# Dhia-naouali/dinov3-jax

Measured on NVIDIA H100. Metric: global_crops_per_sec, higher is better.
Workload: dtype bf16

## Files before the change

### dinov3-jax_b200/csrc/attention.cu

```cuda
#include "ptx.cuh"
#include <climits>
#include <cstdlib>
#include "d3_internal.h"

namespace d3 {

constexpr float LOG2E = 1.4426950408889634f;
constexpr int SMEM_ALIGN = 1024;

__device__ __forceinline__ uint8_t* smem_base_1024(uint8_t* raw) {
  return reinterpret_cast<uint8_t*>((reinterpret_cast<uintptr_t>(raw) + 1023) & ~uintptr_t(1023));
}

struct AttnShape {
  int G;
  int span;
  int n_crops;
  int N;
  int nkb;
  int D;
  int H;
  float scale;
  const float* sin_t;
  const float* cos_t;
  int prefix;
};

__device__ __forceinline__ uint32_t sw128_offset(int row, int col) {
  return (uint32_t)(row * 128 + ((((col >> 3) ^ (row & 7)) & 7) << 4) + (col & 7) * 2);
}

struct RowInfo { int g, klo, khi; bool ok; };
__device__ __forceinline__ RowInfo row_info(const AttnShape& sh, int c, int q) {
  RowInfo ri;
  ri.g = min(q / sh.N, sh.G - 1);
  ri.klo = ri.g * sh.N;
  ri.khi = ri.klo + sh.N;
  ri.ok = (q < sh.span) && (c * sh.G + ri.g < sh.n_crops);
  return ri;
}

template <int NI, int NO>
__device__ __forceinline__ void online_softmax(float (&s)[4 * NI], float (&o)[NO], float (&m)[2], float (&l)[2],
                                               const RowInfo (&ri)[2], int k0, int c2, float cs) {
  const int kb0 = k0 + c2;
  const bool full = k0 >= max(ri[0].klo, ri[1].klo) && k0 + 8 * NI <= min(ri[0].khi, ri[1].khi);
  float mx[2] = {-3.0e38f, -3.0e38f};
#pragma unroll
  for (int i = 0; i < NI; ++i)
#pragma unroll
    for (int j = 0; j < 4; ++j) {
      const int hh = j >> 1, kk = kb0 + 8 * i + (j & 1);
      if (full || (kk >= ri[hh].klo && kk < ri[hh].khi)) mx[hh] = fmaxf(mx[hh], s[4 * i + j]);
    }
  float corr[2], ms[2];
#pragma unroll
  for (int hh = 0; hh < 2; ++hh) {
    mx[hh] = fmaxf(mx[hh], __shfl_xor_sync(0xffffffffu, mx[hh], 1));
    mx[hh] = fmaxf(mx[hh], __shfl_xor_sync(0xffffffffu, mx[hh], 2));
    const float mn = fmaxf(m[hh], mx[hh]);
    corr[hh] = ex2_approx((m[hh] - mn) * cs);
    m[hh] = mn;
    ms[hh] = mn * cs;
    l[hh] *= corr[hh];
  }
#pragma unroll
  for (int i = 0; i < NI; ++i)
#pragma unroll
    for (int j = 0; j < 4; ++j) {
      const int hh = j >> 1, kk = kb0 + 8 * i + (j & 1);
      const float p = (full || (kk >= ri[hh].klo && kk < ri[hh].khi)) ? ex2_approx(fmaf(s[4 * i + j], cs, -ms[hh])) : 0.f;
      s[4 * i + j] = p;
      l[hh] += p;
      if (i < NO / 4) o[4 * i + j] *= corr[hh];
    }
}

template <int NO>
__device__ __forceinline__ void store_o_lse(const float (&o)[NO], float (&l)[2], const float (&m)[2], const RowInfo (&ri)[2],
                                            const AttnShape& sh, int c, int h, int row_base, int wq0, int r_in, int c2,
                                            __nv_bfloat16* O, float* LSE) {
#pragma unroll
  for (int hh = 0; hh < 2; ++hh) {
    l[hh] += __shfl_xor_sync(0xffffffffu, l[hh], 1);
    l[hh] += __shfl_xor_sync(0xffffffffu, l[hh], 2);
    const int q = wq0 + r_in + 8 * hh;
    if (!ri[hh].ok) continue;
    const float inv = 1.f / l[hh];
    __nv_bfloat16* dst = O + (size_t)(row_base + q) * sh.D + h * (2 * NO) + c2;
#pragma unroll
    for (int i = 0; i < NO / 4; ++i)
      *reinterpret_cast<uint32_t*>(dst + 8 * i) = pack_bf16(o[4 * i + 2 * hh] * inv, o[4 * i + 2 * hh + 1] * inv);
    if (LSE && c2 == 0)
      LSE[((size_t)(c * sh.G + ri[hh].g) * sh.H + h) * sh.N + (q - ri[hh].klo)] = m[hh] * sh.scale + logf(l[hh]);
  }
}

__host__ __device__ constexpr int fwd_smem(int nkb) { return SMEM_ALIGN + 16384 + 2 * nkb * 8192 + 8; }

__global__ void __launch_bounds__(256)
attn_fwd_kernel(const __grid_constant__ CUtensorMap tmQ, const __grid_constant__ CUtensorMap tmKV,
                __nv_bfloat16* __restrict__ O, float* __restrict__ LSE, const AttnShape sh) {
  extern __shared__ uint8_t smem_raw[];
  uint8_t* sQ = smem_base_1024(smem_raw);
  uint8_t* sK = sQ + 16384;
  uint8_t* sV = sK + sh.nkb * 8192;
  uint64_t* bar = reinterpret_cast<uint64_t*>(sV + sh.nkb * 8192);

// ... 264 lines not shown
  const uint64_t kd = gmma_desc_sw128(smem_u32(sK), 16, 1024);
  const uint64_t vd = gmma_desc_sw128(smem_u32(sV), 16, 1024);
  wgmma_fence();
#pragma unroll
  for (int k = 0; k < 4; ++k) {
    wgmma_m64n128k16_ss<0, 0>(s, qd + 2 * k, kd + 2 * k, k > 0 ? 1u : 0u);
    wgmma_m64n128k16_ss<0, 0>(dp, dod + 2 * k, vd + 2 * k, k > 0 ? 1u : 0u);
  }
  wgmma_commit();
  wgmma_wait<0>();
  fence_regs(s);
  fence_regs(dp);
#pragma unroll
  for (int hh = 0; hh < 2; ++hh) {
    const int q = q0 + r_in + 8 * hh;
    const RowInfo ri = row_info(sh, c, q);
    float lse2, dl;
    row_stats(sh, LSE, Delta, c, h, q, lse2, dl);
    const int lo = ri.ok ? ri.klo - kt * 128 : 0, hi = ri.ok ? ri.khi - kt * 128 : 0;
#pragma unroll
    for (int i = 0; i < 16; ++i)
#pragma unroll
      for (int j = 0; j < 2; ++j) {
        const int e = 4 * i + 2 * hh + j, col = 8 * i + c2 + j;
        const bool ok = col >= lo && col < hi;
        const float p = ok ? ex2_approx(fmaf(s[e], cs, -lse2)) : 0.f;
        dp[e] = ok ? (p * sh.scale) * (dp[e] - dl) : 0.f;
        s[e] = p;
      }
  }
}

__device__ __forceinline__ void stash_p_ds(const float (&s)[64], const float (&dp)[64], uint8_t* sP, uint8_t* sDS, int row,
                                           int c2) {
#pragma unroll
  for (int hh = 0; hh < 2; ++hh) {
#pragma unroll
    for (int i = 0; i < 16; ++i) {
      const uint32_t off = (i >> 3) * 16384 + sw128_offset(row + 8 * hh, (8 * i + c2) & 63);
      *reinterpret_cast<uint32_t*>(sP + off) = pack_bf16(s[4 * i + 2 * hh], s[4 * i + 2 * hh + 1]);
      *reinterpret_cast<uint32_t*>(sDS + off) = pack_bf16(dp[4 * i + 2 * hh], dp[4 * i + 2 * hh + 1]);
    }
  }
}

__device__ __forceinline__ void dkdv_mma(float (&dk)[32], float (&dv)[32], const uint8_t* sP, const uint8_t* sDS,
                                         const uint8_t* sDOt, const uint8_t* sQt, int wg) {
  const uint64_t pd = gmma_desc_sw128(smem_u32(sP + wg * 16384), 16384, 1024);
  const uint64_t sd = gmma_desc_sw128(smem_u32(sDS + wg * 16384), 16384, 1024);
  const uint64_t dod = gmma_desc_sw128(smem_u32(sDOt), 8192, 1024);
  const uint64_t qd = gmma_desc_sw128(smem_u32(sQt), 8192, 1024);
  fence_regs(dk);
  fence_regs(dv);
  wgmma_fence();
#pragma unroll
  for (int k = 0; k < 8; ++k) {
    wgmma_m64n64k16_ss<1, 1>(dv, pd + 128 * k, dod + 128 * k, 1u);
    wgmma_m64n64k16_ss<1, 1>(dk, sd + 128 * k, qd + 128 * k, 1u);
  }
  wgmma_commit();
  wgmma_wait<0>();
  fence_regs(dk);
  fence_regs(dv);
}

__device__ __forceinline__ void dq_mma(float (&dq)[32], const float (&dp)[64], const uint8_t* sK) {
  uint32_t a[8][4];
#pragma unroll
  for (int kk = 0; kk < 8; ++kk)
#pragma unroll
    for (int e = 0; e < 4; ++e) a[kk][e] = pack_bf16(dp[8 * kk + 2 * e], dp[8 * kk + 2 * e + 1]);
  const uint64_t kd = gmma_desc_sw128(smem_u32(sK), 8192, 1024);
  fence_regs(dq);
  wgmma_fence();
#pragma unroll
  for (int kk = 0; kk < 8; ++kk) wgmma_m64n64k16_rs<1>(dq, a[kk], kd + 128 * kk, 1u);
  wgmma_commit();
  wgmma_wait<0>();
  fence_regs(dq);
}


__host__ __device__ constexpr int bwd_fused_smem(int n_t) {
  return n_t * 32768 * 2 + 32768 + (n_t > 1 ? 2 * 32768 : 0) + n_t * 128 * 8 + 2 * n_t * 8;
}

__device__ __forceinline__ uint64_t desc_here(const void* p, uint32_t lbo, uint32_t sbo) {
  uint32_t a;
  asm volatile("mov.b32 %0, %1;" : "=r"(a) : "r"(smem_u32(p)));
  return gmma_desc_sw128(a, lbo, sbo);
}

template <int R>
__device__ __forceinline__ void fence_frag(uint32_t (&a)[R][4]) {
#pragma unroll
  for (int i = 0; i < R; ++i)
#pragma unroll
    for (int e = 0; e < 4; ++e) asm volatile("" : "+r"(a[i][e])::"memory");
}

__global__ void __launch_bounds__(256, 1)
attn_bwd_fused_kernel(const __grid_constant__ CUtensorMap tmQKV, const __grid_constant__ CUtensorMap tmDO,
                      const float* __restrict__ LSE, const float* __restrict__ Delta, __nv_bfloat16* __restrict__ dQKV,
                      const AttnShape sh) {
  extern __shared__ __align__(1024) uint8_t smem_al[];
  const int nT = (sh.span + 127) / 128;
  uint8_t* sKV = smem_al;
  uint8_t* sQDO = sKV + nT * 32768;
  uint8_t* sDS = sQDO + nT * 32768;
  uint8_t* sDS0 = sDS + 32768;
  float* sDQ = reinterpret_cast<float*>(sDS0 + 32768);
  float* sLSE = reinterpret_cast<float*>(sDS + (nT > 1 ? 3 * 32768 : 32768));
  float* sDel = sLSE + nT * 128;
  uint64_t* bar_kv = reinterpret_cast<uint64_t*>(sDel + nT * 128);
  uint64_t* bar_q = bar_kv + nT;

  const int wg = threadIdx.x >> 7, t = threadIdx.x & 127;
  const int r_in = 16 * (t >> 5) + ((t & 31) >> 2), c2 = 2 * (t & 3);
  const int h = blockIdx.x, c = blockIdx.y;
  const int row_base = c * sh.span;
  if (threadIdx.x == 0) {
    tma_prefetch_desc(&tmQKV);
    tma_prefetch_desc(&tmDO);
    for (int i = 0; i < 2 * nT; ++i) mbar_init(bar_kv + i, 1);
    fence_mbar_init();
  }
  __syncthreads();
  if (threadIdx.x < 32 && elect_one()) {
    for (int i = 0; i < nT; ++i) {
      mbar_expect_tx(bar_kv + i, 32768);
      tma_load_2d(&tmQKV, bar_kv + i, sKV + i * 32768, sh.D + h * 64, row_base + i * 128);
      tma_load_2d(&tmQKV, bar_kv + i, sKV + i * 32768 + 16384, 2 * sh.D + h * 64, row_base + i * 128);
      mbar_expect_tx(bar_q + i, 32768);
      tma_load_2d(&tmQKV, bar_q + i, sQDO + i * 32768, h * 64, row_base + i * 128);
      tma_load_2d(&tmDO, bar_q + i, sQDO + i * 32768 + 16384, h * 64, row_base + i * 128);
    }
  }
  for (int q = threadIdx.x; q < nT * 128; q += 256) {
    const RowInfo ri = row_info(sh, c, q);
    const size_t stat = ((size_t)(c * sh.G + ri.g) * sh.H + h) * sh.N + (q - ri.klo);
    sLSE[q] = ri.ok ? LSE[stat] * LOG2E : 0.f;
    sDel[q] = ri.ok ? Delta[stat] : 0.f;
  }
  __syncthreads();

  const float cs = sh.scale * LOG2E;
  int pair = 0;
#pragma unroll 1
  for (int kt = 0; kt < nT; ++kt) {
    mbar_wait(bar_kv + kt, 0);
    const uint8_t* sK = sKV + kt * 32768;
    const uint8_t* sV = sK + 16384;
    int lo[2], hi[2];
#pragma unroll
    for (int hh = 0; hh < 2; ++hh) {
      const RowInfo ri = row_info(sh, c, kt * 128 + wg * 64 + r_in + 8 * hh);
      lo[hh] = ri.ok ? ri.klo : 0;
      hi[hh] = ri.ok ? ri.khi : 0;
    }
    float dk[32], dv[32];
#pragma unroll 1
    for (int qt = 0; qt < nT; ++qt, ++pair) {
      mbar_wait(bar_q + qt, 0);
      const uint8_t* sQt = sQDO + qt * 32768;
      const uint8_t* sDOt = sQt + 16384;
      const bool defer = nT == 2 && kt == 0 && qt == 0;
      uint8_t* stash = defer ? sDS0 : sDS;
      uint32_t pa[2][4][4], da[2][4][4];
#pragma unroll
      for (int hf = 0; hf < 2; ++hf) {
        float s[32], dp[32];
        {
          const uint64_t kd = desc_here(sK + wg * 8192, 16, 1024);
          const uint64_t vd = desc_here(sV + wg * 8192, 16, 1024);
          const uint64_t qd = desc_here(sQt + hf * 8192, 16, 1024);
          const uint64_t dod = desc_here(sDOt + hf * 8192, 16, 1024);
          wgmma_fence();
#pragma unroll
          for (int k = 0; k < 4; ++k) {
            wgmma_m64n64k16_ss<0, 0>(s, kd + 2 * k, qd + 2 * k, k > 0 ? 1u : 0u);
            wgmma_m64n64k16_ss<0, 0>(dp, vd + 2 * k, dod + 2 * k, k > 0 ? 1u : 0u);
          }
          wgmma_commit();
          wgmma_wait<0>();
          fence_regs(s);
          fence_regs(dp);
          if (hf == 1) { fence_frag(pa[0]); fence_frag(da[0]); }
        }
        const float* lse2 = sLSE + qt * 128 + hf * 64;
        const float* del = sDel + qt * 128 + hf * 64;
#pragma unroll
        for (int i = 0; i < 8; ++i) {
          const int col = 8 * i + c2;
          const float2 l2 = *reinterpret_cast<const float2*>(lse2 + col);
          const float2 dl = *reinterpret_cast<const float2*>(del + col);
          const int q = qt * 128 + hf * 64 + col;
          float pv[4], dv4[4];
#pragma unroll
          for (int j = 0; j < 4; ++j) {
            const int hh = j >> 1, qq = q + (j & 1);
            const bool ok = qq >= lo[hh] && qq < hi[hh];
            const float p = ok ? ex2_approx(fmaf(s[4 * i + j], cs, -((j & 1) ? l2.y : l2.x))) : 0.f;
            dv4[j] = ok ? (p * sh.scale) * (dp[4 * i + j] - ((j & 1) ? dl.y : dl.x)) : 0.f;
            pv[j] = p;
          }
          pa[hf][i >> 1][2 * (i & 1)] = pack_bf16(pv[0], pv[1]);
          pa[hf][i >> 1][2 * (i & 1) + 1] = pack_bf16(pv[2], pv[3]);
          da[hf][i >> 1][2 * (i & 1)] = pack_bf16(dv4[0], dv4[1]);
          da[hf][i >> 1][2 * (i & 1) + 1] = pack_bf16(dv4[2], dv4[3]);
        }
        if (hf == 0 && pair > 1) named_bar_sync(1, 256);
#pragma unroll
        for (int hh = 0; hh < 2; ++hh)
#pragma unroll
          for (int i = 0; i < 8; ++i) {
            const uint32_t off = hf * 16384 + sw128_offset(wg * 64 + r_in + 8 * hh, 8 * i + c2);
            *reinterpret_cast<uint32_t*>(stash + off) = da[hf][i >> 1][2 * (i & 1) + hh];
          }
        {
          const uint64_t dod = desc_here(sDOt, 8192, 1024);
          const uint64_t qd = desc_here(sQt, 8192, 1024);
          const uint32_t acc_on = (qt > 0 || hf > 0) ? 1u : 0u;
          if (acc_on) { fence_regs(dk); fence_regs(dv); }
          wgmma_fence();
#pragma unroll
          for (int kk = 0; kk < 4; ++kk) {
            const int ks = 4 * hf + kk;
            wgmma_m64n64k16_rs<1>(dv, pa[hf][kk], dod + 128 * ks, (acc_on || kk > 0) ? 1u : 0u);
            wgmma_m64n64k16_rs<1>(dk, da[hf][kk], qd + 128 * ks, (acc_on || kk > 0) ? 1u : 0u);
          }
          wgmma_commit();
        }
      }
      fence_proxy_async_smem();
      if (defer) {
        wgmma_wait<0>();
        fence_regs(dk);
        fence_regs(dv);
        fence_frag(pa[1]);
        fence_frag(da[1]);
        continue;
      }
      named_bar_sync(2, 256);
      const bool from_partial = nT == 2 && kt == 1 && qt == 1;
      float dq[32];
      float4* part = reinterpret_cast<float4*>(sDQ) + wg * 8 * 128 + t;
      if (from_partial) {
#pragma unroll
        for (int j = 0; j < 8; ++j) {
          const float4 v = part[j * 128];
          dq[4 * j] = v.x; dq[4 * j + 1] = v.y; dq[4 * j + 2] = v.z; dq[4 * j + 3] = v.w;
        }
      }
      {
        const uint64_t sd = desc_here(sDS + wg * 16384, 16384, 1024);
        const uint64_t kbd = desc_here(sK, 8192, 1024);
        fence_regs(dq);
        wgmma_fence();
#pragma unroll
        for (int kk = 0; kk < 8; ++kk)
          wgmma_m64n64k16_ss<1, 1>(dq, sd + 128 * kk, kbd + 128 * kk, (from_partial || kk > 0) ? 1u : 0u);
        if (nT == 2 && kt == 1 && qt == 0) {
          const uint64_t sd0 = desc_here(sDS0 + wg * 16384, 16384, 1024);
          const uint64_t k0d = desc_here(sKV, 8192, 1024);
#pragma unroll
          for (int kk = 0; kk < 8; ++kk) wgmma_m64n64k16_ss<1, 1>(dq, sd0 + 128 * kk, k0d + 128 * kk, 1u);
        }
        wgmma_commit();
        wgmma_wait<0>();
        fence_regs(dq);
        fence_regs(dk);
        fence_regs(dv);
        fence_frag(pa[1]);
        fence_frag(da[1]);
      }
      if (nT == 2 && kt == 0) {
#pragma unroll
        for (int j = 0; j < 8; ++j) part[j * 128] = make_float4(dq[4 * j], dq[4 * j + 1], dq[4 * j + 2], dq[4 * j + 3]);
      } else {
        store_grad_rows(dq, sh, c, row_base, qt * 128 + wg * 64, r_in, c2, h, 0, true, dQKV);
      }
    }
    store_grad_rows(dk, sh, c, row_base, kt * 128 + wg * 64, r_in, c2, h, 1, true, dQKV);
    store_grad_rows(dv, sh, c, row_base, kt * 128 + wg * 64, r_in, c2, h, 2, false, dQKV);
  }
}

using DkdvRing = TileRing<DKDV_STAGES, 32768>;
constexpr int DKDV_SMEM = SMEM_ALIGN + 2 * 16384 + 2 * 32768 + DkdvRing::SMEM + 8;
using DqRing = TileRing<DQ_STAGES, 32768>;
constexpr int DQ_SMEM = SMEM_ALIGN + 2 * 16384 + DqRing::SMEM + 8;

__global__ void __launch_bounds__(RING_THREADS, 1)
attn_bwd_dkdv_kernel(const __grid_constant__ CUtensorMap tmQKV, const __grid_constant__ CUtensorMap tmDO,
                     const float* __restrict__ LSE, const float* __restrict__ Delta, __nv_bfloat16* __restrict__ dQKV,
                     const AttnShape sh) {
  extern __shared__ uint8_t smem_raw[];
  uint8_t* sK = smem_base_1024(smem_raw);
  uint8_t* sV = sK + 16384;
  uint8_t* sP = sV + 16384;
  uint8_t* sDS = sP + 32768;
  const DkdvRing ring(sDS + 32768);
  uint64_t* bar_kv = ring.end();

  const int wg = threadIdx.x >> 7, t = threadIdx.x & 127;
  const int r_in = 16 * (t >> 5) + ((t & 31) >> 2), c2 = 2 * (t & 3);
  const int kt = blockIdx.x, h = blockIdx.y, c = blockIdx.z;
  const int row_base = c * sh.N, nq = (sh.N + 127) >> 7;
  if (threadIdx.x == 0) {
    tma_prefetch_desc(&tmQKV);
    tma_prefetch_desc(&tmDO);
    ring.init(8);
    mbar_init(bar_kv, 1);
    fence_mbar_init();
  }
  __syncthreads();
  if (ring_producer(wg, [&] {
        mbar_expect_tx(bar_kv, 32768);
        tma_load_2d(&tmQKV, bar_kv, sK, sh.D + h * 64, row_base + kt * 128);
        tma_load_2d(&tmQKV, bar_kv, sV, 2 * sh.D + h * 64, row_base + kt * 128);
        ring.fill(nq, [&](uint64_t* bar, uint8_t* dst, int qt) {
          tma_load_2d(&tmQKV, bar, dst, h * 64, row_base + qt * 128);
          tma_load_2d(&tmDO, bar, dst + 16384, h * 64, row_base + qt * 128);
        });
      }))
    return;
  mbar_wait(bar_kv, 0);
  float dk[32], dv[32];
#pragma unroll
  for (int i = 0; i < 32; ++i) { dk[i] = 0.f; dv[i] = 0.f; }
#pragma unroll 1
  for (int qt = 0; qt < nq; ++qt) {
    const uint8_t* sQt = ring.wait(qt);
    const uint8_t* sDOt = sQt + 16384;
    float s[64], dp[64];
    p_ds_tile(sh, LSE, Delta, c, h, qt * 128 + wg * 64, kt, sQt + wg * 8192, sDOt + wg * 8192, sK, sV, r_in, c2, s, dp);
    stash_p_ds(s, dp, sP, sDS, wg * 64 + r_in, c2);
    fence_proxy_async_smem();
    named_bar_sync(1, 256);
    dkdv_mma(dk, dv, sP, sDS, sDOt, sQt, wg);
    ring.release(qt);
    named_bar_sync(1, 256);
  }
  store_grad_rows(dk, sh, c, row_base, kt * 128 + wg * 64, r_in, c2, h, 1, true, dQKV);
  store_grad_rows(dv, sh, c, row_base, kt * 128 + wg * 64, r_in, c2, h, 2, false, dQKV);
}

__global__ void __launch_bounds__(RING_THREADS, 1)
attn_bwd_dq_kernel(const __grid_constant__ CUtensorMap tmQKV, const __grid_constant__ CUtensorMap tmDO,
                   const float* __restrict__ LSE, const float* __restrict__ Delta, __nv_bfloat16* __restrict__ dQKV,
                   const AttnShape sh) {
  extern __shared__ uint8_t smem_raw[];
  uint8_t* sQ = smem_base_1024(smem_raw);
  uint8_t* sDO = sQ + 16384;
  const DqRing ring(sDO + 16384);
  uint64_t* bar_q = ring.end();

  const int wg = threadIdx.x >> 7, t = threadIdx.x & 127;
  const int r_in = 16 * (t >> 5) + ((t & 31) >> 2), c2 = 2 * (t & 3);
  const int qt = blockIdx.x, h = blockIdx.y, c = blockIdx.z;
  const int q0 = qt * 128, row_base = c * sh.N, nk = (sh.N + 127) >> 7;
  const int n_wg = (q0 + 64 < sh.N) ? 2 : 1;
  if (threadIdx.x == 0) {
    tma_prefetch_desc(&tmQKV);
    tma_prefetch_desc(&tmDO);
    ring.init(4 * n_wg);
    mbar_init(bar_q, 1);
// ... 261 lines not shown
  int lo[2], hi[2];
#pragma unroll
  for (int hh = 0; hh < 2; ++hh) {
    const RowInfo ri = row_info(sh, c, wq0 + r_in + 8 * hh);
    row_stats(sh, LSE, Delta, c, h, wq0 + r_in + 8 * hh, lse2[hh], dl[hh]);
    lo[hh] = ri.ok ? ri.klo : 0;
    hi[hh] = ri.ok ? ri.khi : 0;
  }
  const float cs = sh.scale * LOG2E;
  float dq[64];
#pragma unroll
  for (int i = 0; i < 64; ++i) dq[i] = 0.f;
#pragma unroll 1
  for (int kt = 0; kt < nk; ++kt) {
    const uint8_t* sK = ring.wait(kt);
    const uint8_t* sV = sK + 32768;
#pragma unroll 1
    for (int hf = 0; hf < 2; ++hf) {
      float s[32], dp[32];
      wgmma_fence();
#pragma unroll
      for (int k = 0; k < 8; ++k) {
        wgmma_m64n64k16_ss<0, 0>(s, kdesc128(sQ + wg * 8192, k), kdesc128(sK + hf * 8192, k), k > 0 ? 1u : 0u);
        wgmma_m64n64k16_ss<0, 0>(dp, kdesc128(sDO + wg * 8192, k), kdesc128(sV + hf * 8192, k), k > 0 ? 1u : 0u);
      }
      wgmma_commit();
      wgmma_wait<0>();
      fence_regs(s);
      fence_regs(dp);
      uint32_t da[4][4];
#pragma unroll
      for (int i = 0; i < 8; ++i) {
        const int key = kt * 128 + hf * 64 + 8 * i + c2;
        float d4[4];
#pragma unroll
        for (int j = 0; j < 4; ++j) {
          const int hh = j >> 1, kk = key + (j & 1);
          const bool ok = kk >= lo[hh] && kk < hi[hh];
          const float p = ok ? ex2_approx(fmaf(s[4 * i + j], cs, -lse2[hh])) : 0.f;
          d4[j] = ok ? (p * sh.scale) * (dp[4 * i + j] - dl[hh]) : 0.f;
        }
        da[i >> 1][2 * (i & 1)] = pack_bf16(d4[0], d4[1]);
        da[i >> 1][2 * (i & 1) + 1] = pack_bf16(d4[2], d4[3]);
      }
      const uint64_t kd = desc_here(sK + hf * 8192, 16384, 1024);
      fence_regs(dq);
      wgmma_fence();
#pragma unroll
      for (int kk = 0; kk < 4; ++kk) wgmma_m64n128k16_rs<1>(dq, da[kk], kd + 128 * kk, 1u);
      wgmma_commit();
      wgmma_wait<0>();
      fence_regs(dq);
      fence_frag(da);
    }
    ring.release(kt);
  }
  store_grad_rows(dq, sh, c, row_base, wq0, r_in, c2, h, 0, true, dQKV);
}

static int make_map(CUtensorMap* map, const void* ptr, long rows, int cols, int ld, int box_rows) {
  cuuint64_t dims[2] = {(cuuint64_t)cols, (cuuint64_t)rows};
  cuuint64_t strides[1] = {(cuuint64_t)ld * 2};
  cuuint32_t box[2] = {64, (cuuint32_t)box_rows};
  cuuint32_t estr[2] = {1, 1};
  return encode_tensor_map_2d_bf16(map, ptr, dims, strides, box, estr);
}

constexpr int ATTN_MAX_TOKENS = 32768;
constexpr int ATTN_FWD_RESIDENT_SPAN = 448;
constexpr int ATTN_BWD_RESIDENT_SPAN = 256;

static int attn_shape(AttnShape* s, int n_crops, int N, int D, int H) {
  if (D != H * 64 && D != H * 128) return set_error(D3_ERR_ARG, "attention: head_dim must be 64 or 128");
  if (N <= 0 || n_crops <= 0) return set_error(D3_ERR_ARG, "attention: empty problem");
  if (N > ATTN_MAX_TOKENS) return set_error(D3_ERR_ARG, "attention: N > 32768 tokens per crop");
  if ((long)n_crops * N > INT_MAX) return set_error(D3_ERR_ARG, "attention: n_crops * N must be below 2^31 token rows");
  s->N = N; s->D = D; s->H = H; s->n_crops = n_crops;
  s->scale = (D == H * 64) ? 0.125f : 0.08838834764831845f;
  s->sin_t = nullptr; s->cos_t = nullptr; s->prefix = 0;
  s->G = (N <= 64) ? (128 / N) : 1;
  if (s->G > n_crops) s->G = n_crops;
  s->span = s->G * N;
  s->nkb = (s->span + 63) / 64;
  return D3_OK;
}

static int tile_grid(const AttnShape& s, dim3* grid) {
  const int groups = (s.n_crops + s.G - 1) / s.G;
  if (s.H > 65535 || groups > 65535) return set_error(D3_ERR_ARG, "attention: H and crop groups must be <= 65535");
  *grid = dim3((s.span + 127) / 128, s.H, groups);
  return D3_OK;
}

template <auto kernel, class... Args>
static int launch(dim3 grid, int threads, int smem, int smem_max, cudaStream_t st, const Args&... args) {
  static const cudaError_t cfg = cudaFuncSetAttribute(kernel, cudaFuncAttributeMaxDynamicSharedMemorySize, smem_max);
  (void)cfg;
  kernel<<<grid, threads, smem, st>>>(args...);
  D3_CHECK_LAUNCH();
  return D3_OK;
}

}

using namespace d3;

extern "C" {

int d3_attn_fwd(const void* qkv, void* o, float* lse, int n_crops, int N, int D, int H, void* stream) {
  AttnShape s;
  int rc = attn_shape(&s, n_crops, N, D, H);
  if (rc) return rc;
  dim3 grid;
  if ((rc = tile_grid(s, &grid))) return rc;
  const long T = (long)n_crops * N;
  cudaStream_t st = reinterpret_cast<cudaStream_t>(stream);
  __nv_bfloat16* out = (__nv_bfloat16*)o;
  CUtensorMap tqkv;
  if ((rc = make_map(&tqkv, qkv, T, 3 * D, 3 * D, 128))) return rc;
  if (D == H * 128)
    return launch<attn_fwd_hd128_kernel>(grid, RING_THREADS, HD128_FWD_SMEM, HD128_FWD_SMEM, st, tqkv, out, lse, s);
  if (s.span > ATTN_FWD_RESIDENT_SPAN)
    return launch<attn_fwd_stream_kernel>(grid, RING_THREADS, FWD_STREAM_SMEM, FWD_STREAM_SMEM, st, tqkv, out, lse, s);
  CUtensorMap tkv;
  if ((rc = make_map(&tkv, qkv, T, 3 * D, 3 * D, 64))) return rc;
  return launch<attn_fwd_kernel>(grid, 256, fwd_smem(s.nkb), fwd_smem((ATTN_FWD_RESIDENT_SPAN + 63) / 64), st, tqkv, tkv,
                                 out, lse, s);
}

int d3_attn_bwd(const void* qkv, const void* o, const void* d_o, const float* lse, float* delta_scratch, void* dqkv,
                int n_crops, int N, int D, int H, const float* rope_sin, const float* rope_cos, int rope_prefix,
                void* stream) {
  AttnShape s;
  int rc = attn_shape(&s, n_crops, N, D, H);
  if (rc) return rc;
  if ((rope_sin == nullptr) != (rope_cos == nullptr)) return set_error(D3_ERR_ARG, "d3_attn_bwd: sin/cos tables");
  if (!delta_scratch) return set_error(D3_ERR_ARG, "d3_attn_bwd: delta scratch buffer");
  const bool hd128 = D == H * 128;
  const bool streamed = s.span > ATTN_BWD_RESIDENT_SPAN;
  dim3 grid;
  if ((hd128 || streamed) && (rc = tile_grid(s, &grid))) return rc;
  s.sin_t = rope_sin; s.cos_t = rope_cos; s.prefix = rope_prefix;
  const long T = (long)n_crops * N;
  cudaStream_t st = reinterpret_cast<cudaStream_t>(stream);
  const long threads = T * (D / 8);
  if (hd128)
    attn_delta_kernel<128><<<(int)((threads + 255) / 256), 256, 0, st>>>((const __nv_bfloat16*)o, (const __nv_bfloat16*)d_o,
                                                                       delta_scratch, T, N, D, H);
  else
    attn_delta_kernel<64><<<(int)((threads + 255) / 256), 256, 0, st>>>((const __nv_bfloat16*)o, (const __nv_bfloat16*)d_o,
                                                                      delta_scratch, T, N, D, H);
  D3_CHECK_LAUNCH();
  CUtensorMap tqkv, tdo;
  if ((rc = make_map(&tqkv, qkv, T, 3 * D, 3 * D, 128))) return rc;
  if ((rc = make_map(&tdo, d_o, T, D, D, 128))) return rc;
  __nv_bfloat16* dq = (__nv_bfloat16*)dqkv;
  if (hd128) {
    if ((rc = launch<attn_bwd_dkdv_hd128_kernel>(grid, RING_THREADS, HD128_BWD_SMEM, HD128_BWD_SMEM, st, tqkv, tdo, lse,
                                                 delta_scratch, dq, s)))
      return rc;
    return launch<attn_bwd_dq_hd128_kernel>(grid, RING_THREADS, HD128_BWD_SMEM, HD128_BWD_SMEM, st, tqkv, tdo, lse,
                                            delta_scratch, dq, s);
  }
  if (streamed) {
    if ((rc = launch<attn_bwd_dkdv_kernel>(grid, RING_THREADS, DKDV_SMEM, DKDV_SMEM, st, tqkv, tdo, lse, delta_scratch, dq,
                                           s)))
      return rc;
    return launch<attn_bwd_dq_kernel>(grid, RING_THREADS, DQ_SMEM, DQ_SMEM, st, tqkv, tdo, lse, delta_scratch, dq, s);
  }
  return launch<attn_bwd_fused_kernel>(dim3(H, (n_crops + s.G - 1) / s.G), 256, bwd_fused_smem((s.span + 127) / 128),
                                       bwd_fused_smem(ATTN_BWD_RESIDENT_SPAN / 128), st, tqkv, tdo, lse, delta_scratch,
                                       dq, s);
}

}
```

Measured before the change: 550.0.

## Make fused attention backward persistent with double-buffered TMA prefetch of next item

The fused backward kernel becomes persistent: it launches at most one CTA per SM (by occupancy) and loops over (head, crop-group) items. Tile shared memory is fixed at two 64KB slots, so the next item's K/V/Q/dO tiles are TMA-loaded while the current one is computed. The next item's LSE/Delta stats are staged with cp.async. This is meant to hide per-CTA load latency and launch tail, at the cost of extra barriers, parity tracking and more complex slot reuse logic.

```diff
diff --git a/dinov3-jax_b200/csrc/attention.cu b/dinov3-jax_b200/csrc/attention.cu
--- a/dinov3-jax_b200/csrc/attention.cu
+++ b/dinov3-jax_b200/csrc/attention.cu
@@ -1,4 +1,5 @@
 #include "ptx.cuh"
+#include <algorithm>
 #include <climits>
 #include <cstdlib>
 #include "d3_internal.h"
@@ -24,6 +25,7 @@
   const float* sin_t;
   const float* cos_t;
   int prefix;
+  int items;
 };
 
 __device__ __forceinline__ uint32_t sw128_offset(int row, int col) {
@@ -454,7 +456,7 @@
 
 
 __host__ __device__ constexpr int bwd_fused_smem(int n_t) {
-  return n_t * 32768 * 2 + 32768 + (n_t > 1 ? 2 * 32768 : 0) + n_t * 128 * 8 + 2 * n_t * 8;
+  return 2 * 65536 + 32768 + (n_t > 1 ? 2 * 32768 : 0) + n_t * 128 * 8 + 2 * 8;
 }
 
 __device__ __forceinline__ uint64_t desc_here(const void* p, uint32_t lbo, uint32_t sbo) {
@@ -469,6 +471,38 @@
   for (int i = 0; i < R; ++i)
 #pragma unroll
     for (int e = 0; e < 4; ++e) asm volatile("" : "+r"(a[i][e])::"memory");
+}
+
+__device__ __forceinline__ void bwd_load_tile(const CUtensorMap* tmQKV, const CUtensorMap* tmDO, const AttnShape& sh,
+                                              int item, int tile, uint8_t* dst, uint64_t* bar) {
+  const int h = item % sh.H, row = (item / sh.H) * sh.span + tile * 128;
+  mbar_expect_tx(bar, 65536);
+  tma_load_2d(tmQKV, bar, dst, sh.D + h * 64, row);
+  tma_load_2d(tmQKV, bar, dst + 16384, 2 * sh.D + h * 64, row);
+  tma_load_2d(tmQKV, bar, dst + 32768, h * 64, row);
+  tma_load_2d(tmDO, bar, dst + 49152, h * 64, row);
+}
+
+__device__ __forceinline__ void bwd_stage_stats(const AttnShape& sh, const float* __restrict__ LSE,
+                                                const float* __restrict__ Delta, int item, int nT, float* sLSE,
+                                                float* sDel) {
+  const int h = item % sh.H, c = item / sh.H;
+  for (int q = threadIdx.x; q < nT * 128; q += 256) {
+    const RowInfo ri = row_info(sh, c, q);
+    const size_t stat = ((size_t)(c * sh.G + ri.g) * sh.H + h) * sh.N + (q - ri.klo);
+    if (ri.ok) {
+      cp_async_4(sLSE + q, LSE + stat);
+      cp_async_4(sDel + q, Delta + stat);
+    } else {
+      sLSE[q] = 0.f;
+      sDel[q] = 0.f;
+    }
+  }
+}
+
+__device__ __forceinline__ void bwd_stats_land(int nT, float* sLSE) {
+  cp_async_wait_all();
+  for (int q = threadIdx.x; q < nT * 128; q += 256) sLSE[q] *= LOG2E;
 }
 
 __global__ void __launch_bounds__(256, 1)
@@ -477,184 +511,195 @@
                       const AttnShape sh) {
   extern __shared__ __align__(1024) uint8_t smem_al[];
   const int nT = (sh.span + 127) / 128;
-  uint8_t* sKV = smem_al;
-  uint8_t* sQDO = sKV + nT * 32768;
-  uint8_t* sDS = sQDO + nT * 32768;
+  uint8_t* sT = smem_al;
+  uint8_t* sDS = sT + 2 * 65536;
   uint8_t* sDS0 = sDS + 32768;
   float* sDQ = reinterpret_cast<float*>(sDS0 + 32768);
   float* sLSE = reinterpret_cast<float*>(sDS + (nT > 1 ? 3 * 32768 : 32768));
   float* sDel = sLSE + nT * 128;
-  uint64_t* bar_kv = reinterpret_cast<uint64_t*>(sDel + nT * 128);
-  uint64_t* bar_q = bar_kv + nT;
+  uint64_t* bar = reinterpret_cast<uint64_t*>(sDel + nT * 128);
 
   const int wg = threadIdx.x >> 7, t = threadIdx.x & 127;
   const int r_in = 16 * (t >> 5) + ((t & 31) >> 2), c2 = 2 * (t & 3);
-  const int h = blockIdx.x, c = blockIdx.y;
-  const int row_base = c * sh.span;
   if (threadIdx.x == 0) {
     tma_prefetch_desc(&tmQKV);
     tma_prefetch_desc(&tmDO);
-    for (int i = 0; i < 2 * nT; ++i) mbar_init(bar_kv + i, 1);
+    mbar_init(bar, 1);
+    mbar_init(bar + 1, 1);
     fence_mbar_init();
   }
   __syncthreads();
-  if (threadIdx.x < 32 && elect_one()) {
-    for (int i = 0; i < nT; ++i) {
-      mbar_expect_tx(bar_kv + i, 32768);
-      tma_load_2d(&tmQKV, bar_kv + i, sKV + i * 32768, sh.D + h * 64, row_base + i * 128);
-      tma_load_2d(&tmQKV, bar_kv + i, sKV + i * 32768 + 16384, 2 * sh.D + h * 64, row_base + i * 128);
-      mbar_expect_tx(bar_q + i, 32768);
-      tma_load_2d(&tmQKV, bar_q + i, sQDO + i * 32768, h * 64, row_base + i * 128);
-      tma_load_2d(&tmDO, bar_q + i, sQDO + i * 32768 + 16384, h * 64, row_base + i * 128);
-    }
-  }
-  for (int q = threadIdx.x; q < nT * 128; q += 256) {
-    const RowInfo ri = row_info(sh, c, q);
-    const size_t stat = ((size_t)(c * sh.G + ri.g) * sh.H + h) * sh.N + (q - ri.klo);
-    sLSE[q] = ri.ok ? LSE[stat] * LOG2E : 0.f;
-    sDel[q] = ri.ok ? Delta[stat] : 0.f;
-  }
-  __syncthreads();
+  if (threadIdx.x == 0) {
+    bwd_load_tile(&tmQKV, &tmDO, sh, blockIdx.x, 0, sT, bar);
+    if (nT == 2) bwd_load_tile(&tmQKV, &tmDO, sh, blockIdx.x, 1, sT + 65536, bar + 1);
+    else if (blockIdx.x + gridDim.x < sh.items)
+      bwd_load_tile(&tmQKV, &tmDO, sh, blockIdx.x + gridDim.x, 0, sT + 65536, bar + 1);
+  }
+  bwd_stage_stats(sh, LSE, Delta, blockIdx.x, nT, sLSE, sDel);
 
   const float cs = sh.scale * LOG2E;
-  int pair = 0;
 #pragma unroll 1
-  for (int kt = 0; kt < nT; ++kt) {
-    mbar_wait(bar_kv + kt, 0);
-    const uint8_t* sK = sKV + kt * 32768;
-    const uint8_t* sV = sK + 16384;
-    int lo[2], hi[2];
-#pragma unroll
-    for (int hh = 0; hh < 2; ++hh) {
-      const RowInfo ri = row_info(sh, c, kt * 128 + wg * 64 + r_in + 8 * hh);
-      lo[hh] = ri.ok ? ri.klo : 0;
-      hi[hh] = ri.ok ? ri.khi : 0;
-    }
-    float dk[32], dv[32];
+  for (int it = 0; blockIdx.x + it * gridDim.x < sh.items; ++it) {
+    const int item = blockIdx.x + it * gridDim.x, next = item + gridDim.x;
+    const int h = item % sh.H, c = item / sh.H;
+    const int row_base = c * sh.span;
+    const uint32_t par = (nT == 1 ? it >> 1 : it) & 1;
+    bwd_stats_land(nT, sLSE);
+    __syncthreads();
+    int pair = 0;
 #pragma unroll 1
-    for (int qt = 0; qt < nT; ++qt, ++pair) {
-      mbar_wait(bar_q + qt, 0);
-      const uint8_t* sQt = sQDO + qt * 32768;
-      const uint8_t* sDOt = sQt + 16384;
-      const bool defer = nT == 2 && kt == 0 && qt == 0;
-      uint8_t* stash = defer ? sDS0 : sDS;
-      uint32_t pa[2][4][4], da[2][4][4];
-#pragma unroll
-      for (int hf = 0; hf < 2; ++hf) {
-        float s[32], dp[32];
+    for (int kt = 0; kt < nT; ++kt) {
+      const int kslot = nT == 1 ? (it & 1) : kt;
+      mbar_wait(bar + kslot, par);
+      const uint8_t* sK = sT + kslot * 65536;
+      const uint8_t* sV = sK + 16384;
+      int lo[2], hi[2];
+#pragma unroll
+      for (int hh = 0; hh < 2; ++hh) {
+        const RowInfo ri = row_info(sh, c, kt * 128 + wg * 64 + r_in + 8 * hh);
+        lo[hh] = ri.ok ? ri.klo : 0;
+        hi[hh] = ri.ok ? ri.khi : 0;
+      }
+      float dk[32], dv[32];
+#pragma unroll 1
+      for (int qt = 0; qt < nT; ++qt, ++pair) {
+        const int qslot = nT == 1 ? (it & 1) : qt;
+        mbar_wait(bar + qslot, par);
+        const uint8_t* sQt = sT + qslot * 65536 + 32768;
+        const uint8_t* sDOt = sQt + 16384;
+        const bool defer = nT == 2 && kt == 0 && qt == 0;
+        uint8_t* stash = defer ? sDS0 : sDS;
+        uint32_t pa[2][4][4], da[2][4][4];
+#pragma unroll
+        for (int hf = 0; hf < 2; ++hf) {
+          float s[32], dp[32];
+          {
+            const uint64_t kd = desc_here(sK + wg * 8192, 16, 1024);
+            const uint64_t vd = desc_here(sV + wg * 8192, 16, 1024);
+            const uint64_t qd = desc_here(sQt + hf * 8192, 16, 1024);
+            const uint64_t dod = desc_here(sDOt + hf * 8192, 16, 1024);
+            wgmma_fence();
+#pragma unroll
+            for (int k = 0; k < 4; ++k) {
+              wgmma_m64n64k16_ss<0, 0>(s, kd + 2 * k, qd + 2 * k, k > 0 ? 1u : 0u);
+              wgmma_m64n64k16_ss<0, 0>(dp, vd + 2 * k, dod + 2 * k, k > 0 ? 1u : 0u);
+            }
+            wgmma_commit();
+            wgmma_wait<0>();
+            fence_regs(s);
+            fence_regs(dp);
+            if (hf == 1) { fence_frag(pa[0]); fence_frag(da[0]); }
+          }
+          const float* lse2 = sLSE + qt * 128 + hf * 64;
+          const float* del = sDel + qt * 128 + hf * 64;
+#pragma unroll
+          for (int i = 0; i < 8; ++i) {
+            const int col = 8 * i + c2;
+            const float2 l2 = *reinterpret_cast<const float2*>(lse2 + col);
+            const float2 dl = *reinterpret_cast<const float2*>(del + col);
+            const int q = qt * 128 + hf * 64 + col;
+            float pv[4], dv4[4];
+#pragma unroll
+            for (int j = 0; j < 4; ++j) {
+              const int hh = j >> 1, qq = q + (j & 1);
+              const bool ok = qq >= lo[hh] && qq < hi[hh];
+              const float p = ok ? ex2_approx(fmaf(s[4 * i + j], cs, -((j & 1) ? l2.y : l2.x))) : 0.f;
+              dv4[j] = ok ? (p * sh.scale) * (dp[4 * i + j] - ((j & 1) ? dl.y : dl.x)) : 0.f;
+              pv[j] = p;
+            }
+            pa[hf][i >> 1][2 * (i & 1)] = pack_bf16(pv[0], pv[1]);
+            pa[hf][i >> 1][2 * (i & 1) + 1] = pack_bf16(pv[2], pv[3]);
+            da[hf][i >> 1][2 * (i & 1)] = pack_bf16(dv4[0], dv4[1]);
+            da[hf][i >> 1][2 * (i & 1) + 1] = pack_bf16(dv4[2], dv4[3]);
+          }
+          if (hf == 0 && pair > 1) {
+            named_bar_sync(1, 256);
+            if (pair == 3 && threadIdx.x == 0 && next < sh.items) bwd_load_tile(&tmQKV, &tmDO, sh, next, 0, sT, bar);
+          }
+#pragma unroll
+          for (int hh = 0; hh < 2; ++hh)
+#pragma unroll
+            for (int i = 0; i < 8; ++i) {
+              const uint32_t off = hf * 16384 + sw128_offset(wg * 64 + r_in + 8 * hh, 8 * i + c2);
+              *reinterpret_cast<uint32_t*>(stash + off) = da[hf][i >> 1][2 * (i & 1) + hh];
+            }
+          {
+            const uint64_t dod = desc_here(sDOt, 8192, 1024);
+            const uint64_t qd = desc_here(sQt, 8192, 1024);
+            const uint32_t acc_on = (qt > 0 || hf > 0) ? 1u : 0u;
+            if (acc_on) { fence_regs(dk); fence_regs(dv); }
+            wgmma_fence();
+#pragma unroll
+            for (int kk = 0; kk < 4; ++kk) {
+              const int ks = 4 * hf + kk;
+              wgmma_m64n64k16_rs<1>(dv, pa[hf][kk], dod + 128 * ks, (acc_on || kk > 0) ? 1u : 0u);
+              wgmma_m64n64k16_rs<1>(dk, da[hf][kk], qd + 128 * ks, (acc_on || kk > 0) ? 1u : 0u);
+            }
+            wgmma_commit();
+          }
+        }
+        fence_proxy_async_smem();
+        if (defer) {
+          wgmma_wait<0>();
+          fence_regs(dk);
+          fence_regs(dv);
+          fence_frag(pa[1]);
+          fence_frag(da[1]);
+          continue;
+        }
+        named_bar_sync(2, 256);
+        const bool from_partial = nT == 2 && kt == 1 && qt == 1;
+        float dq[32];
+        float4* part = reinterpret_cast<float4*>(sDQ) + wg * 8 * 128 + t;
+        if (from_partial) {
+#pragma unroll
+          for (int j = 0; j < 8; ++j) {
+            const float4 v = part[j * 128];
+            dq[4 * j] = v.x; dq[4 * j + 1] = v.y; dq[4 * j + 2] = v.z; dq[4 * j + 3] = v.w;
+          }
+        }
         {
-          const uint64_t kd = desc_here(sK + wg * 8192, 16, 1024);
-          const uint64_t vd = desc_here(sV + wg * 8192, 16, 1024);
-          const uint64_t qd = desc_here(sQt + hf * 8192, 16, 1024);
-          const uint64_t dod = desc_here(sDOt + hf * 8192, 16, 1024);
+          const uint64_t sd = desc_here(sDS + wg * 16384, 16384, 1024);
+          const uint64_t kbd = desc_here(sK, 8192, 1024);
+          fence_regs(dq);
           wgmma_fence();
 #pragma unroll
-          for (int k = 0; k < 4; ++k) {
-            wgmma_m64n64k16_ss<0, 0>(s, kd + 2 * k, qd + 2 * k, k > 0 ? 1u : 0u);
-            wgmma_m64n64k16_ss<0, 0>(dp, vd + 2 * k, dod + 2 * k, k > 0 ? 1u : 0u);
+          for (int kk = 0; kk < 8; ++kk)
+            wgmma_m64n64k16_ss<1, 1>(dq, sd + 128 * kk, kbd + 128 * kk, (from_partial || kk > 0) ? 1u : 0u);
+          if (nT == 2 && kt == 1 && qt == 0) {
+            const uint64_t sd0 = desc_here(sDS0 + wg * 16384, 16384, 1024);
+            const uint64_t k0d = desc_here(sT, 8192, 1024);
+#pragma unroll
+            for (int kk = 0; kk < 8; ++kk) wgmma_m64n64k16_ss<1, 1>(dq, sd0 + 128 * kk, k0d + 128 * kk, 1u);
           }
           wgmma_commit();
           wgmma_wait<0>();
-          fence_regs(s);
-          fence_regs(dp);
-          if (hf == 1) { fence_frag(pa[0]); fence_frag(da[0]); }
+          fence_regs(dq);
+          fence_regs(dk);
+          fence_regs(dv);
+          fence_frag(pa[1]);
+          fence_frag(da[1]);
         }
-        const float* lse2 = sLSE + qt * 128 + hf * 64;
-        const float* del = sDel + qt * 128 + hf * 64;
-#pragma unroll
-        for (int i = 0; i < 8; ++i) {
-          const int col = 8 * i + c2;
-          const float2 l2 = *reinterpret_cast<const float2*>(lse2 + col);
-          const float2 dl = *reinterpret_cast<const float2*>(del + col);
-          const int q = qt * 128 + hf * 64 + col;
-          float pv[4], dv4[4];
-#pragma unroll
-          for (int j = 0; j < 4; ++j) {
-            const int hh = j >> 1, qq = q + (j & 1);
-            const bool ok = qq >= lo[hh] && qq < hi[hh];
-            const float p = ok ? ex2_approx(fmaf(s[4 * i + j], cs, -((j & 1) ? l2.y : l2.x))) : 0.f;
-            dv4[j] = ok ? (p * sh.scale) * (dp[4 * i + j] - ((j & 1) ? dl.y : dl.x)) : 0.f;
-            pv[j] = p;
+        if (kt == nT - 1 && qt == nT - 1) {
+          __syncthreads();
+          if (threadIdx.x == 0) {
+            if (nT == 1 && next + gridDim.x < sh.items)
+              bwd_load_tile(&tmQKV, &tmDO, sh, next + gridDim.x, 0, sT + (it & 1) * 65536, bar + (it & 1));
+            else if (nT == 2 && next < sh.items)
+              bwd_load_tile(&tmQKV, &tmDO, sh, next, 1, sT + 65536, bar + 1);
           }
-          pa[hf][i >> 1][2 * (i & 1)] = pack_bf16(pv[0], pv[1]);
-          pa[hf][i >> 1][2 * (i & 1) + 1] = pack_bf16(pv[2], pv[3]);
-          da[hf][i >> 1][2 * (i & 1)] = pack_bf16(dv4[0], dv4[1]);
-          da[hf][i >> 1][2 * (i & 1) + 1] = pack_bf16(dv4[2], dv4[3]);
+          if (next < sh.items) bwd_stage_stats(sh, LSE, Delta, next, nT, sLSE, sDel);
         }
-        if (hf == 0 && pair > 1) named_bar_sync(1, 256);
-#pragma unroll
-        for (int hh = 0; hh < 2; ++hh)
-#pragma unroll
-          for (int i = 0; i < 8; ++i) {
-            const uint32_t off = hf * 16384 + sw128_offset(wg * 64 + r_in + 8 * hh, 8 * i + c2);
-            *reinterpret_cast<uint32_t*>(stash + off) = da[hf][i >> 1][2 * (i & 1) + hh];
-          }
-        {
-          const uint64_t dod = desc_here(sDOt, 8192, 1024);
-          const uint64_t qd = desc_here(sQt, 8192, 1024);
-          const uint32_t acc_on = (qt > 0 || hf > 0) ? 1u : 0u;
-          if (acc_on) { fence_regs(dk); fence_regs(dv); }
-          wgmma_fence();
-#pragma unroll
-          for (int kk = 0; kk < 4; ++kk) {
-            const int ks = 4 * hf + kk;
-            wgmma_m64n64k16_rs<1>(dv, pa[hf][kk], dod + 128 * ks, (acc_on || kk > 0) ? 1u : 0u);
-            wgmma_m64n64k16_rs<1>(dk, da[hf][kk], qd + 128 * ks, (acc_on || kk > 0) ? 1u : 0u);
-          }
-          wgmma_commit();
+        if (nT == 2 && kt == 0) {
+#pragma unroll
+          for (int j = 0; j < 8; ++j) part[j * 128] = make_float4(dq[4 * j], dq[4 * j + 1], dq[4 * j + 2], dq[4 * j + 3]);
+        } else {
+          store_grad_rows(dq, sh, c, row_base, qt * 128 + wg * 64, r_in, c2, h, 0, true, dQKV);
         }
       }
-      fence_proxy_async_smem();
-      if (defer) {
-        wgmma_wait<0>();
-        fence_regs(dk);
-        fence_regs(dv);
-        fence_frag(pa[1]);
-        fence_frag(da[1]);
-        continue;
-      }
-      named_bar_sync(2, 256);
-      const bool from_partial = nT == 2 && kt == 1 && qt == 1;
-      float dq[32];
-      float4* part = reinterpret_cast<float4*>(sDQ) + wg * 8 * 128 + t;
-      if (from_partial) {
-#pragma unroll
-        for (int j = 0; j < 8; ++j) {
-          const float4 v = part[j * 128];
-          dq[4 * j] = v.x; dq[4 * j + 1] = v.y; dq[4 * j + 2] = v.z; dq[4 * j + 3] = v.w;
-        }
-      }
-      {
-        const uint64_t sd = desc_here(sDS + wg * 16384, 16384, 1024);
-        const uint64_t kbd = desc_here(sK, 8192, 1024);
-        fence_regs(dq);
-        wgmma_fence();
-#pragma unroll
-        for (int kk = 0; kk < 8; ++kk)
-          wgmma_m64n64k16_ss<1, 1>(dq, sd + 128 * kk, kbd + 128 * kk, (from_partial || kk > 0) ? 1u : 0u);
-        if (nT == 2 && kt == 1 && qt == 0) {
-          const uint64_t sd0 = desc_here(sDS0 + wg * 16384, 16384, 1024);
-          const uint64_t k0d = desc_here(sKV, 8192, 1024);
-#pragma unroll
-          for (int kk = 0; kk < 8; ++kk) wgmma_m64n64k16_ss<1, 1>(dq, sd0 + 128 * kk, k0d + 128 * kk, 1u);
-        }
-        wgmma_commit();
-        wgmma_wait<0>();
-        fence_regs(dq);
-        fence_regs(dk);
-        fence_regs(dv);
-        fence_frag(pa[1]);
-        fence_frag(da[1]);
-      }
-      if (nT == 2 && kt == 0) {
-#pragma unroll
-        for (int j = 0; j < 8; ++j) part[j * 128] = make_float4(dq[4 * j], dq[4 * j + 1], dq[4 * j + 2], dq[4 * j + 3]);
-      } else {
-        store_grad_rows(dq, sh, c, row_base, qt * 128 + wg * 64, r_in, c2, h, 0, true, dQKV);
-      }
+      store_grad_rows(dk, sh, c, row_base, kt * 128 + wg * 64, r_in, c2, h, 1, true, dQKV);
+      store_grad_rows(dv, sh, c, row_base, kt * 128 + wg * 64, r_in, c2, h, 2, false, dQKV);
     }
-    store_grad_rows(dk, sh, c, row_base, kt * 128 + wg * 64, r_in, c2, h, 1, true, dQKV);
-    store_grad_rows(dv, sh, c, row_base, kt * 128 + wg * 64, r_in, c2, h, 2, false, dQKV);
   }
 }
 
@@ -1082,6 +1127,9 @@
   if (s->G > n_crops) s->G = n_crops;
   s->span = s->G * N;
   s->nkb = (s->span + 63) / 64;
+  const long items = (long)H * ((n_crops + s->G - 1) / s->G);
+  if (items > INT_MAX) return set_error(D3_ERR_ARG, "attention: H * crop groups must be below 2^31");
+  s->items = (int)items;
   return D3_OK;
 }
 
@@ -1097,6 +1145,20 @@
   static const cudaError_t cfg = cudaFuncSetAttribute(kernel, cudaFuncAttributeMaxDynamicSharedMemorySize, smem_max);
   (void)cfg;
   kernel<<<grid, threads, smem, st>>>(args...);
+  D3_CHECK_LAUNCH();
+  return D3_OK;
+}
+
+template <auto kernel, class... Args>
+static int launch_persistent(long items, int threads, int smem, int smem_max, cudaStream_t st, const Args&... args) {
+  static const cudaError_t cfg = cudaFuncSetAttribute(kernel, cudaFuncAttributeMaxDynamicSharedMemorySize, smem_max);
+  if (cfg != cudaSuccess) return set_error(D3_ERR_CUDA, cudaGetErrorString(cfg));
+  int per_sm = 0;
+  const cudaError_t e = cudaOccupancyMaxActiveBlocksPerMultiprocessor(&per_sm, kernel, threads, smem);
+  if (e != cudaSuccess) return set_error(D3_ERR_CUDA, cudaGetErrorString(e));
+  if (per_sm < 1) return set_error(D3_ERR_CUDA, "attention: a persistent CTA does not fit on an SM");
+  const long grid = std::min<long>(items, (long)per_sm * sm_count());
+  kernel<<<(unsigned)grid, threads, smem, st>>>(args...);
   D3_CHECK_LAUNCH();
   return D3_OK;
 }
@@ -1168,9 +1230,9 @@
       return rc;
     return launch<attn_bwd_dq_kernel>(grid, RING_THREADS, DQ_SMEM, DQ_SMEM, st, tqkv, tdo, lse, delta_scratch, dq, s);
   }
-  return launch<attn_bwd_fused_kernel>(dim3(H, (n_crops + s.G - 1) / s.G), 256, bwd_fused_smem((s.span + 127) / 128),
-                                       bwd_fused_smem(ATTN_BWD_RESIDENT_SPAN / 128), st, tqkv, tdo, lse, delta_scratch,
-                                       dq, s);
-}
-
-}
+  return launch_persistent<attn_bwd_fused_kernel>(s.items, 256, bwd_fused_smem((s.span + 127) / 128),
+                                                  bwd_fused_smem(ATTN_BWD_RESIDENT_SPAN / 128), st, tqkv, tdo, lse,
+                                                  delta_scratch, dq, s);
+}
+
+}
```

After: 550.4, median of 6. No clear change (+0.1%).
